# rgl-epfl/large-steps-pytorch

Measured on NVIDIA H100. Metric: from_differential solves/sec @1M verts, higher is better.
Workload: dtype f32

## Files before the change

include/largesteps_b200_diag.h:

```cpp
#ifndef LARGESTEPS_B200_DIAG_H
#define LARGESTEPS_B200_DIAG_H

#include "largesteps_b200.h"

#ifdef __cplusplus
extern "C" {
#endif

int ls_pcg_bench_spmm(void *handle, int k, int launches, void *stream);
int ls_pcg_bench(void **handles, int n_handles, int k, int which, int launches, void *stream);
int ls_pcg_batch_plan(int n, const int32_t *nslices, const int32_t *pat, int max_smem, int32_t *cluster, int32_t *res,
                      int32_t *group, int32_t *n_groups);
int ls_pcg_batch_plan_ex(int n, const int32_t *nslices, const int32_t *pat, const int32_t *cheb, int max_smem,
                         int32_t *cluster, int32_t *res, int32_t *group, int32_t *n_groups);
int ls_pcg_plan(int nslices, int k, int pat, int precond, int sm_count, int max_smem, int coop, int64_t *out8);
int ls_pcg_pattern_copy(void *handle, int64_t *info4, int32_t *poff, uint32_t *words, void *stream);
int ls_pcg_phase_cycles(void *handle, int64_t *out, int n , void *stream);

#ifdef __cplusplus
}
#endif
#endif
```

large-steps-pytorch_b200/csrc/ls_pcg.cu:

```cuda
#include <new>
#include <string.h>
#include <stdlib.h>
#include "ls_spmm_host.h"
#include "ls_sell_kernel.cuh"
#include "ls_pcg_fused.cuh"
#include "ls_fused_inst.h"

#ifndef LS_CLRES_DEFAULT
#define LS_CLRES_DEFAULT 0
#endif

namespace {

constexpr int KMAX = 4;
constexpr int VEC_THREADS = 256;
constexpr int CHUNK = 8;

struct PcgCtrl {
    double rz[KMAX], pAp[KMAX], rr[KMAX], bb[KMAX];
    float beta[KMAX];
    float rtol2;
    int maxit;
    int it;
    int done;
// ... 28 lines not shown
    int *desc_cnt;
    int *perm;
    int *inv;
    int *scan;
    int has_perm;
    int planned;
    int *soff;
    int2 *ent;
    long long sell_cap;
    long long sell_entries;
    int nslices;
    int sell_on;
    int sell_grid;
    int *poff;
    unsigned int *pcol;
    unsigned char *pcls;
    unsigned long long *pcls_tab;
    unsigned int *patmm;
    long long pat_cap;
    float offc;
    int pat_on;
    int pat_shared;
    int pat_stored;
    int pat_words;
    lsf::GridBar *gbar;
    double *partials;
    long long *dbg;
    unsigned long long *ring;
    int ring_slots;
    float *pv;
    float *z2, *cy, *cd;
    int cheb_m;
    float cheb_c0, cheb_c1[8], cheb_c2[8];
    float *gersh;
    struct FusedCfg : FusedPlan {
        int pat;
        const void *fn, *fn_prof;
    } fused[2];
    int max_smem_optin;
    int refine;
    float theta;
    int sell_tma;
    int sell_pf;
    cudaGraphExec_t graph[KMAX + 1];
    cudaStream_t cap_stream;
    int *pinned_done;
    cudaEvent_t ev[2];
    size_t ws_bytes;
};

static bool want_pattern() {
    const char *e = getenv("LS_PCG_PATTERN");
    return !(e && e[0] == '0');
}

struct Carve {
    size_t off = 0;
    size_t take(size_t bytes) {
        size_t o = off;
// ... 647 lines not shown
    return LS_OK;
}

const void *fused_fn(int K, int res, int nw, int pat, int sync, int prof, int cheb = 0) {
    if (cheb) return (K == 3 && !prof) ? ls_fused_fn_cheb(res, nw, pat, sync) : nullptr;
    if (K == 3 && !prof) return ls_fused_fn_jacobi(res, nw, pat, sync);
    return ls_fused_fn_misc(K, res, nw, pat, sync, prof);
}

static int env_int(const char *name, int dflt) {
    const char *e = getenv(name);
    return (e && e[0]) ? atoi(e) : dflt;
}

constexpr int CLRES_CS = 16;

struct PlanEnv {
    int graph;
    int cluster;
    int res;
    int onecta;
    int clres;
    int small_cta;
};

PlanEnv plan_env() {
    const char *mode = getenv("LS_PCG_MODE"), *small = getenv("LS_PCG_SMALLCTA");
    PlanEnv e;
    e.graph = mode && (mode[0] == 'g' || mode[0] == 'G');
    e.cluster = env_int("LS_PCG_CLUSTER", -1);
    e.res = env_int("LS_PCG_RES", -1);
    e.onecta = env_int("LS_PCG_ONECTA", lsf::PWARPS);
    e.clres = env_int("LS_PCG_CLRES", LS_CLRES_DEFAULT);
    e.small_cta = !(small && small[0] == '0');
    return e;
}

int slices_per_cta(int K, int res, int pat, int cheb, int sync, int max_smem) {
    if (res == 0) return 1 << 30;
    int n = 0;
    while (lsf::fused_smem_bytes(K, res, n + 1, pat, cheb, sync) <= (size_t)max_smem) ++n;
    return n;
}

int auto_precond(int nslices, int sm_count, int max_smem, const PlanEnv &env) {
    if (nslices <= env.onecta) return 1;
    if (env.cluster != 0 && nslices <= env.clres) return 1;
    const int g = sm_count < nslices ? sm_count : nslices;
    const int nsl_max = (nslices + g - 1) / g;
    const bool fits = lsf::fused_smem_bytes(3, 2, nsl_max, 0, 1, 0) + (size_t)nsl_max * 32 * 4 <= (size_t)max_smem;
    return fits ? 2 : 1;
}

FusedPlan plan_fused(int nslices, int K, int pat, int cheb, int sm_count, int max_smem, int coop, const PlanEnv &env) {
    FusedPlan p{};
    if (env.graph) return p;
    const int W = lsf::PWARPS;
// ... 9 lines not shown
        const bool res3 = cs == 1 && K == 3 && !cheb && nsl_max <= slices_per_cta(K, 3, pat, cheb, 1, max_smem);
        int res = (res3 && !(env.res >= 0 && env.res < 3)) ? 3 : 2;
        int nw = W;
        int cap4 = slices_per_cta(K, 4, pat, cheb, 1, max_smem);
        if (cap4 > 63) cap4 = 63;
        if (cs > 1 && !cheb && nsl_max <= cap4 && !(env.res >= 0 && env.res < 4)) {
            res = 4;
            if (K == 3 && nsl_max <= lsf::PT_SMALL / 32 && env.small_cta) nw = lsf::PT_SMALL / 32;
        }
        if (res == 4 && !fused_fn(K, res, nw, pat, 1, 0, cheb)) { res = 2; nw = W; }
        if (fused_fn(K, res, nw, pat, 1, 0, cheb)) return {1, cs, cs, res, nw, 1, nsl_max, lsf::fused_smem_bytes(K, res, nsl_max, pat, cheb, 1)};
    }
    if (!coop) return p;
    int g = sm_count < nslices ? sm_count : nslices;
    if (g > 255) g = 255;
    if (g < 1) g = 1;
    const int nsl_max = (nslices + g - 1) / g;
    int res = nsl_max <= slices_per_cta(K, 2, pat, cheb, 0, max_smem) ? 2 : (nsl_max <= slices_per_cta(K, 1, pat, cheb, 0, max_smem) ? 1 : 0);
    if (env.res >= 0 && env.res < res) res = env.res;
    int nw = W;
    if (K == 3 && res == 2 && nsl_max <= 16 && env.small_cta) nw = lsf::PT_SMALL / 32;
    if (!fused_fn(K, res, nw, pat, 0, 0, cheb)) return p;
    return {1, g, 0, res, nw, 0, nsl_max, lsf::fused_smem_bytes(K, res, nsl_max, pat, cheb, 0)};
}

cudaLaunchConfig_t cluster_launch(int grid, int cluster, int threads, size_t smem, cudaStream_t stream, cudaLaunchAttribute *at) {
    cudaLaunchConfig_t lc = {};
    lc.gridDim = dim3(grid);
    lc.blockDim = dim3(threads);
    lc.dynamicSmemBytes = smem;
    lc.stream = stream;
    at->id = cudaLaunchAttributeClusterDimension;
    at->val.clusterDim.x = cluster;
    at->val.clusterDim.y = 1;
    at->val.clusterDim.z = 1;
    lc.attrs = at;
    lc.numAttrs = 1;
    return lc;
}

bool device_accepts(const void *fn, const FusedPlan &p, const LsDevInfo &di) {
    bool ok = cudaFuncSetAttribute(fn, cudaFuncAttributeMaxDynamicSharedMemorySize, di.max_smem_optin) == cudaSuccess;
    if (ok && p.cluster > 8) ok = cudaFuncSetAttribute(fn, cudaFuncAttributeNonPortableClusterSizeAllowed, 1) == cudaSuccess;
    if (ok && p.cluster > 1) {
        cudaLaunchAttribute at;
        const cudaLaunchConfig_t lc = cluster_launch(p.grid, p.cluster, p.nw * 32, p.smem, 0, &at);
// ... 8 lines not shown
    return ok;
}

void configure_fused(PcgHandle *h, const LsDevInfo &di, const PlanEnv &env, int K, PcgHandle::FusedCfg *c) {
    memset(c, 0, sizeof(*c));
    if (!h->sell_on) return;
    const int cheb = (K == 3 && h->cheb_m > 1) ? 1 : 0;
    const int pat = (K == 3 && h->pat_on) ? 1 : 0;
    int coop = 0;
    if (cudaDeviceGetAttribute(&coop, cudaDevAttrCooperativeLaunch, di.device) != cudaSuccess) {
        coop = 0;
        cudaGetLastError();
    }
    auto kernel = [&](const FusedPlan &q, int prof) { return fused_fn(K, q.res, q.nw, pat, q.sync, prof, cheb); };
    FusedPlan p = plan_fused(h->nslices, K, pat, cheb, di.sm_count, di.max_smem_optin, coop, env);
    if (p.on && p.sync == 1 && !device_accepts(kernel(p, 0), p, di)) {
        PlanEnv grid_only = env;
        grid_only.cluster = 0;
        p = plan_fused(h->nslices, K, pat, cheb, di.sm_count, di.max_smem_optin, coop, grid_only);
    }
    if (!p.on || (p.sync == 0 && !device_accepts(kernel(p, 0), p, di))) return;
    static_cast<FusedPlan &>(*c) = p;
    c->pat = pat;
    c->fn = kernel(p, 0);
    c->fn_prof = kernel(p, 1);
    if (c->fn_prof) {
        cudaFuncSetAttribute(c->fn_prof, cudaFuncAttributeMaxDynamicSharedMemorySize, di.max_smem_optin);
        if (p.cluster > 8) cudaFuncSetAttribute(c->fn_prof, cudaFuncAttributeNonPortableClusterSizeAllowed, 1);
    }
    cudaGetLastError();
}

void fused_handle_args(const PcgHandle *h, int nsl_max, lsf::FusedArgs &a) {
    a.V = (int)h->V;
    a.Vp = h->Vp;
    a.nslices = h->nslices;
    a.nsl_max = nsl_max;
    a.soff = h->soff;
    a.ent = h->ent;
    a.poff = h->poff;
    a.pcol = h->pcol;
    a.pcls = h->pcls;
    a.pcls_tab = h->pcls_tab;
    a.offc = h->offc;
    a.pat_l1 = h->pat_shared;
    a.dinv = h->dinv;
// ... 2 lines not shown
    a.r = h->r;
    a.s = h->Ap;
    a.z = h->p;
    a.z2 = h->z2;
    a.cy = h->cy;
    a.cd = h->cd;
    a.perm = h->has_perm ? h->perm : nullptr;
    a.refine = h->refine;
    a.theta = h->theta;
    a.cheb_m = h->cheb_m;
    a.cheb_c0 = h->cheb_c0;
    for (int j = 0; j < 8; ++j) {
        a.cheb_c1[j] = h->cheb_c1[j];
        a.cheb_c2[j] = h->cheb_c2[j];
    }
}

int solve_fused(PcgHandle *h, const float *b, float *x, const float *x0, int k, float rtol, int maxit, float *info_dev,
                float *info_host, cudaStream_t stream) {
    PcgHandle::FusedCfg &c = h->fused[k == 4 ? 1 : 0];
    lsf::FusedArgs a{};
    fused_handle_args(h, c.nsl_max, a);
    a.kb = k;
    if (k == 4) a.cheb_m = 0;
    a.b = b;
    a.out = x;
    a.x0 = x0;
    a.rtol = rtol;
    a.maxit = maxit;
    a.bar = h->gbar;
    a.partials = h->partials;
    a.info = info_dev ? info_dev : h->info;
    const bool prof = getenv("LS_PCG_PROFILE") != nullptr && c.fn_prof != nullptr;
    a.dbg = prof ? h->dbg : nullptr;
    const void *fn = prof ? c.fn_prof : c.fn;
    void *params[] = {(void *)&a};
    cudaError_t ce;
    if (c.sync == 1) {
        if (c.cluster > 1) {
            cudaLaunchAttribute at;
            const cudaLaunchConfig_t lc = cluster_launch(c.grid, c.cluster, c.nw * 32, c.smem, stream, &at);
            ce = cudaLaunchKernelExC(&lc, fn, params);
        } else {
            ce = cudaLaunchKernel(fn, dim3(1), dim3(c.nw * 32), params, c.smem, stream);
        }
    } else {
// ... 306 lines not shown
            TRY_OR_FAIL(cudaGetLastError());
            lsk::pat_share_copy_kernel<<<2 * di.sm_count, 256, 0, stream>>>(ns, h->poff, h->pcol, npoff,
                                                                              reinterpret_cast<const unsigned int *>(h->p), soff2, stats, cap_scr);
            g_ls_launches.fetch_add(1);
            TRY_OR_FAIL(cudaGetLastError());
        }
        int hover = 1, hst[2] = {ns, 0}, hwords = 0;
        TRY_OR_FAIL(cudaMemcpyAsync(&hover, over, sizeof(int), cudaMemcpyDeviceToHost, stream));
        if (cap_scr > 0) {
            TRY_OR_FAIL(cudaMemcpyAsync(hst, stats, sizeof(int), cudaMemcpyDeviceToHost, stream));
            TRY_OR_FAIL(cudaMemcpyAsync(&hst[1], soff2 + ns, sizeof(int), cudaMemcpyDeviceToHost, stream));
        }
        TRY_OR_FAIL(cudaMemcpyAsync(&hwords, h->poff + ns, sizeof(int), cudaMemcpyDeviceToHost, stream));
        TRY_OR_FAIL(cudaStreamSynchronize(stream));
        h->pat_on = hover ? 0 : 1;
        h->pat_shared = (h->pat_on && cap_scr > 0 && lsk::pat_share_on(ns, hst[0], hst[1], cap_scr)) ? 1 : 0;
        h->pat_stored = h->pat_shared ? hst[0] : ns;
        h->pat_words = hwords;
        if (cap_scr > 0) {
            TRY_OR_FAIL(cudaMemsetAsync(h->r, 0, (size_t)((char *)(ptab + pmask + 1) - (char *)h->r), stream));
            if (lsk::pat_share_on(ns, hst[0], hst[1], cap_scr)) TRY_OR_FAIL(cudaMemsetAsync(h->p, 0, (size_t)hst[1] * 4, stream));
        }
    }
    h->cheb_m = 0;
    if (precond == 2 && hgersh > 0.f) {
        int m = env_int("LS_PCG_CHEB_M", 4);
        if (m < 2) m = 2;
        if (m > 8) m = 8;
        const double b = 1.02 * (double)hgersh, a = b / 30.0;
        const double th = 0.5 * (b + a), de = 0.5 * (b - a), sg = th / de;
        double rho = 1.0 / sg;
        h->cheb_c0 = (float)(1.0 / th);
        for (int j = 1; j < m; ++j) {
            const double rn = 1.0 / (2.0 * sg - rho);
            h->cheb_c1[j - 1] = (float)(rn * rho);
            h->cheb_c2[j - 1] = (float)(2.0 * rn / de);
            rho = rn;
        }
        h->cheb_m = m;
    }
    configure_fused(h, di, env, 3, &h->fused[0]);
    if (k_max >= 4) configure_fused(h, di, env, 4, &h->fused[1]);
    if (hflags & 8) {
        ls_set_error("perm_new2old is not a permutation of [0, V)");
        return fail(LS_ERR_BAD_ARG);
    }
// ... 165 lines not shown
    out8[0] = h->sell_on;
    out8[1] = h->sell_entries;
    out8[2] = h->sell_on ? h->sell_grid : h->spmm_grid;
    out8[3] = h->vec_grid;
    out8[4] = 0;
    out8[5] = 0;
    out8[6] = h->planned;
    out8[7] = h->has_perm;
    return LS_OK;
}

extern "C" int ls_pcg_plan(int nslices, int k, int pat, int precond, int sm_count, int max_smem, int coop, int64_t *out8) {
    LS_REQUIRE(out8 != nullptr, "out8 is NULL");
    LS_REQUIRE(nslices >= 1, "nslices must be positive");
    LS_REQUIRE(k == 3 || k == 4, "k must be 3 or 4 (the column counts of the fused kernel's instantiations)");
    LS_REQUIRE(precond >= 0 && precond <= 3, "precond must be 0 (none), 1 (Jacobi), 2 (Chebyshev polynomial over Jacobi) or 3 (auto)");
    LS_REQUIRE(sm_count >= 1 && max_smem > 0, "sm_count and max_smem must be positive");
    const PlanEnv env = plan_env();
    if (precond == 3) precond = auto_precond(nslices, sm_count, max_smem, env);
    const int cheb = (k == 3 && precond == 2) ? 1 : 0;
    const FusedPlan p = plan_fused(nslices, k, (k == 3 && pat) ? 1 : 0, cheb, sm_count, max_smem, coop ? 1 : 0, env);
    const int64_t o[8] = {p.on, p.grid, p.cluster, p.res, p.nw * 32, precond, (int64_t)p.smem, p.nsl_max};
    memcpy(out8, o, sizeof(o));
    return LS_OK;
}

extern "C" int ls_pcg_pattern_copy(void *handle, int64_t *info4, int32_t *poff, uint32_t *words, void *stream_) {
    PcgHandle *h = (PcgHandle *)handle;
    LS_REQUIRE(h != nullptr && info4 != nullptr, "NULL pointer");
    info4[0] = h->pat_on;
    info4[1] = h->nslices;
    info4[2] = h->pat_on ? h->pat_stored : 0;
    info4[3] = h->pat_on ? h->pat_words : 0;
    if (h->pat_on && poff != nullptr && words != nullptr) {
        cudaStream_t stream = (cudaStream_t)stream_;
        LS_CUDA_TRY(cudaMemcpyAsync(poff, h->poff, (size_t)(h->nslices + 1) * 4, cudaMemcpyDeviceToHost, stream));
        LS_CUDA_TRY(cudaMemcpyAsync(words, h->pcol, (size_t)h->pat_words * 4, cudaMemcpyDeviceToHost, stream));
        LS_CUDA_TRY(cudaStreamSynchronize(stream));
    }
    return LS_OK;
}

extern "C" int64_t ls_pcg_spmm_bytes(void *handle, int k) {
    PcgHandle *h = (PcgHandle *)handle;
    if (!h) return 0;
    return 8 * h->nnz + 4 * (h->V + 1) + 8 * (int64_t)k * h->V;
// ... 261 lines not shown
```

large-steps-pytorch_b200/csrc/ls_pcg_fused.cuh:

```cuda
#pragma once
#include <cuda_bf16.h>
#include <type_traits>
#include "ls_common.cuh"
#include "ls_sell_kernel.cuh"

#ifndef LS_RING_SOA
#define LS_RING_SOA 0
#endif
#ifndef LS_XP4
#define LS_XP4 0
#endif
#ifndef LS_FHADD
#define LS_FHADD 0
#endif
#ifndef LS_Z_EL
#define LS_Z_EL 0
#endif
#ifndef LS_XP_STREAM
#define LS_XP_STREAM 0
#endif
#ifndef LS_POLL_FENCE
#define LS_POLL_FENCE 0
#endif

namespace lsf {

#ifndef LS_PT
#define LS_PT 768
#endif
constexpr int PT = LS_PT;
constexpr int PWARPS = PT / 32;
constexpr int PT_SMALL = 256;
constexpr int NVMAX = 16;

struct GridBar {
    unsigned int count;
    unsigned int gen;
};

__device__ __forceinline__ unsigned int ld_acquire(const unsigned int *p) {
    unsigned int v;
    asm volatile("ld.acquire.gpu.global.u32 %0, [%1];" : "=r"(v) : "l"(p) : "memory");
    return v;
}
__device__ __forceinline__ float4 ld_coherent4(const float *p) {
    float4 v;
// ... 78 lines not shown
    allreduce_finish<NV>(v, partials, gb, gen, parity, red, G);
}

__device__ __forceinline__ int exp2_of(double d) { return (int)((__double_as_longlong(d) >> 52) & 0x7ff) - 1023; }

template <int KCOL, int N>
__device__ __forceinline__ double pick_lane(const double (&v)[N], int off, int lane) {
    double d = 0.0;
#pragma unroll
    for (int i = 0; i < KCOL; ++i) {
        double t = v[off + i];
        asm volatile("" : "+d"(t));
        if (lane == i) d = t;
    }
    return d;
}

struct FusedArgs {
    int V;
    long long Vp;
    int nslices;
    int nsl_max;
    int kb;
    const int *soff;
    const int2 *ent;
    const int *poff;
    const unsigned int *pcol;
    const unsigned char *pcls;
    const unsigned long long *pcls_tab;
    float offc;
    int pat_l1;
    const float *dinv;
    float *x;
    float *pv;
    float *r;
    float *s;
    float *z;
    float *z2;
    float *cy, *cd;
    int cheb_m;
    float cheb_c0;
    float cheb_c1[8], cheb_c2[8];
    const float *b;
    float *out;
    const float *x0;
    const int *perm;
// ... 297 lines not shown
constexpr size_t FUSED_SMEM_HDR = 4096 + 1024;
constexpr size_t FUSED_BATCH_ARGS = 4352 + 320;
__host__ __device__ inline size_t fused_off_bytes(int nsl_max) { return ((size_t)(2 * (nsl_max + 1)) * 4 + 127) / 128 * 128; }

__host__ __device__ inline int fused_row_bytes(int K, int res, int pat, int cheb = 0) {
    if (res == 0) return 0;
    return 4 * ((res == 1 ? 2 * K : (res == 2 ? 4 * K : 4 * K + 4)) + ((cheb && res == 2) ? 2 * K : 0)) + (pat ? 1 : 4);
}
__host__ __device__ inline size_t fused_tab_bytes(int pat) { return pat ? (size_t)lsk::PAT_CLASSES * 8 : 0; }
__host__ __device__ inline size_t fused_cl_bytes(int sync) { return sync == 1 ? (size_t)(2 * NVMAX * 16 * 8) : 0; }
inline size_t fused_smem_bytes(int K, int res, int nsl_max, int pat, int cheb, int sync) {
    return FUSED_SMEM_HDR + fused_cl_bytes(sync) + fused_off_bytes(nsl_max) + fused_tab_bytes(pat) + (size_t)nsl_max * 32u * fused_row_bytes(K, res, pat, cheb);
}

template <int K, int RES, int NW, bool PAT, int SYNC, bool PROF, bool CHEB = false, bool ZH = false, bool BATCH = false>
__global__ void __launch_bounds__(NW * 32, 1) pcg_fused_kernel(const typename FusedParam<BATCH>::type prm) {
    static_assert(K == 3 || K == 4, "z rows are float4");
    static_assert(!ZH || (K == 3 && !CHEB && RES != 3), "bf16 rows: 3 columns, Jacobi, published through global or distributed shared memory");
    static_assert(RES != 4 || (SYNC == 1 && !CHEB), "cluster-resident rows: one cluster, Jacobi");
    static_assert(!BATCH || (K == 3 && SYNC == 1 && !PROF && (RES == 2 || (RES == 3 && !CHEB))),
                  "batch: one cluster per mesh, 3 columns; Jacobi at RES 3 or 2, Chebyshev at RES 2");
    static_assert(sizeof(Scal) <= FUSED_BATCH_ARGS - 4352 && FUSED_BATCH_ARGS + sizeof(FusedArgs) <= FUSED_SMEM_HDR, "header layout");
    constexpr bool KEEP = (SYNC == 1);
    extern __shared__ __align__(16) unsigned char smem_raw[];
    const FusedArgs &a = kernel_args(prm, smem_raw + FUSED_BATCH_ARGS);
    const bool pkeep = KEEP || (PAT && a.pat_l1 != 0);
    double *red = reinterpret_cast<double *>(smem_raw);
    Scal *S = reinterpret_cast<Scal *>(smem_raw + 4352);
    double *cl = reinterpret_cast<double *>(smem_raw + FUSED_SMEM_HDR);
    int *off_s = reinterpret_cast<int *>(smem_raw + FUSED_SMEM_HDR + fused_cl_bytes(SYNC));
    const int nsl_max = a.nsl_max;
    int *poff_s = off_s + (nsl_max + 1);
    float *tab_d = reinterpret_cast<float *>(reinterpret_cast<unsigned char *>(off_s) + fused_off_bytes(nsl_max));
    float *tab_p = tab_d + lsk::PAT_CLASSES;
    float *r_s = tab_d + (PAT ? 2 * lsk::PAT_CLASSES : 0);
    float *s_s = r_s + (size_t)nsl_max * K * 32;
    float *d_s = s_s + (size_t)nsl_max * K * 32;
    unsigned char *c_s = reinterpret_cast<unsigned char *>(d_s);
    float *x_s = d_s + (size_t)(RES >= 1 ? nsl_max : 0) * (PAT ? 8 : 32);
    float *p_s = x_s + (size_t)nsl_max * K * 32;
    float *z_s = p_s + (size_t)nsl_max * K * 32;
    float *cy_s = z_s;
    float *cd_s = cy_s + (size_t)nsl_max * K * 32;

    const int tid = threadIdx.x, lane = tid & 31, warp = tid >> 5;
    const int G = BATCH ? (int)cluster_nctarank() : (int)gridDim.x, cta = BATCH ? (int)ClusterSync::rank() : (int)blockIdx.x;
    const int s_begin = (RES == 4) ? min(cta * nsl_max, a.nslices) : (int)((long long)a.nslices * cta / G);
    const int s_end = (RES == 4) ? min(s_begin + nsl_max, a.nslices) : (int)((long long)a.nslices * (cta + 1) / G);
    const long long Vp = a.Vp;
    const int kb = a.kb;
    constexpr int U = PAT ? 4 : 8;

    typename std::conditional<SYNC == 1, ClusterSync, GridSync>::type sync;
    if constexpr (SYNC == 1) {
        sync.cl = cl;
        sync.parity = 0;
        sync.G = G;
        sync.red = red;
        sync.S = S;
    } else {
        sync.bar = a.bar;
        sync.partials = a.partials;
        sync.ring = a.ring;
        sync.ring_slots = a.ring_slots;
        sync.gen = 0;
        sync.parity = 0;
        sync.G = G;
        sync.red = red;
        sync.S = S;
    }

    auto R = [&](int li, int k, int row) -> float & { return RES ? r_s[((size_t)li * K + k) * 32 + lane] : a.r[(size_t)k * Vp + row]; };
    auto Sv = [&](int li, int k, int row) -> float & { return RES ? s_s[((size_t)li * K + k) * 32 + lane] : a.s[(size_t)k * Vp + row]; };
    constexpr bool XP4 = (RES == 1) && (LS_XP4 != 0);
// ... 218 lines not shown
                        for (int k = 0; k < K; ++k) w_[k] = fmaf(wv, xk[k], w_[k]);
                    }
                }
                for (int j = U; j < w; j += U) {
#pragma unroll
                    for (int u = 0; u < U; ++u) cv[u] = (j + u < w) ? ld_ent<KEEP>(e + (j + u) * 32) : make_int2(row, 0);
                    float4 xv[U];
#pragma unroll
                    for (int u = 0; u < U; ++u) xv[u] = ZldP(cv[u].x);
#pragma unroll
                    for (int u = 0; u < U; ++u) {
                        const float wv = __int_as_float(cv[u].y);
                        const float xk[4] = {xv[u].x, xv[u].y, xv[u].z, xv[u].w};
                        if (cv[u].x == row) zo = xv[u];
#pragma unroll
                        for (int k = 0; k < K; ++k) w_[k] = fmaf(wv, xk[k], w_[k]);
                    }
                }
            }
            epi(li, row, w_, zo);
        }
    };

    auto own_z = [&](int li, int row) -> float4 {
        if constexpr (CHEB) {
            if constexpr (RES == 2) return make_float4(CY(li, 0), CY(li, 1), CY(li, 2), K > 3 ? CY(li, K > 3 ? 3 : 0) : 0.f);
            else return Zld(row);
        } else if constexpr (RES >= 1) {
            const float di_ = Dv(li, row);
            if constexpr (ZH) return unpack_bf16_row(pack_bf16_row(di_ * R(li, 0, row), di_ * R(li, 1, row), di_ * R(li, 2, row)));
            else return make_float4(di_ * R(li, 0, row), di_ * R(li, 1, row), di_ * R(li, 2, row), K > 3 ? di_ * R(li, K > 3 ? 3 : 0, row) : 0.f);
        } else {
            return ZldP(row);
        }
    };

    auto cheb_first = [&]() {
        for (int s = s_begin + warp; s < s_end; s += NW) {
            const int li = s - s_begin, row = s * 32 + lane;
            const float di = Dv(li, row) * a.cheb_c0;
            float yy[4] = {0.f, 0.f, 0.f, 0.f};
#pragma unroll
            for (int k = 0; k < K; ++k) {
                yy[k] = di * R(li, k, row);
                if constexpr (RES == 2) CY(li, k) = yy[k];
                CD(li, k, row) = yy[k];
            }
            Zst(row, make_float4(yy[0], yy[1], yy[2], yy[3]));
        }
    };
    auto cheb_steps = [&](double (&acc2)[2 * K]) {
// ... 20 lines not shown
                    for (int k = 0; k < K; ++k) {
                        const float rk = R(li, k, row);
                        const float dn = fmaf(c1, dprev[k], c2 * (di * (rk - t[k])));
                        yy[k] = yk[k] + dn;
                        CD(li, k, row) = dn;
                        if constexpr (RES == 2) CY(li, k) = yy[k];
                        if (last) {
                            acc2[k] += (double)rk * (double)yy[k];
                            acc2[K + k] += (double)rk * (double)rk;
                        }
                    }
                    *reinterpret_cast<float4 *>(zalt + 4 * (size_t)row) = make_float4(yy[0], yy[1], yy[2], yy[3]);
                });
            float *tz = zcur;
            zcur = zalt;
            zalt = tz;
        }
    };

    auto cold_init = [&]() {
        double acc[2 * K];
#pragma unroll
        for (int i = 0; i < 2 * K; ++i) acc[i] = 0.0;
        for (int s = s_begin + warp; s < s_end; s += NW) {
            const int li = s - s_begin, row = s * 32 + lane;
            float di = 0.f, bv[K];
#pragma unroll
            for (int k = 0; k < K; ++k) bv[k] = 0.f;
            if (row < a.V) {
                di = a.dinv[row];
                const long long io = a.perm ? a.perm[row] : row;
#pragma unroll
                for (int k = 0; k < K; ++k)
                    if (k < kb) bv[k] = a.b[io * kb + k];
            }
            if (RES && !PAT) d_s[(size_t)li * 32 + lane] = di;
            float zz[4] = {0.f, 0.f, 0.f, 0.f};
#pragma unroll
            for (int k = 0; k < K; ++k) zz[k] = di * bv[k];
            ZstP(row, zz);
#pragma unroll
            for (int k = 0; k < K; ++k) {
                R(li, k, row) = bv[k];
                Sv(li, k, row) = 0.f;
                X(li, k, row) = 0.f;
                P(li, k, row) = 0.f;
// ... 70 lines not shown
                    for (int k = 0; k < K; ++k) {
                        ax[k] = fma((double)wv, (double)xk[k], ax[k]);
                        fl[k] = fmaf(fabsf(wv), fabsf(xk[k]), fl[k]);
                    }
                }
            }
            float di = 0.f, bv[K];
#pragma unroll
            for (int k = 0; k < K; ++k) bv[k] = 0.f;
            if (row < a.V) {
                di = a.dinv[row];
                const long long io = a.perm ? a.perm[row] : row;
#pragma unroll
                for (int k = 0; k < K; ++k)
                    if (k < kb) bv[k] = a.b[io * kb + k];
            }
            if (RES && !PAT) d_s[(size_t)li * 32 + lane] = di;
#pragma unroll
            for (int k = 0; k < K; ++k) {
                const float rv = (float)((double)bv[k] - ax[k]);
                R(li, k, row) = rv;
                float zz = di * rv;
                if constexpr (ZH) zz = __bfloat162float(__float2bfloat16_rn(zz));
                acc[k] += (double)rv * (double)zz;
                acc[K + k] += (double)rv * (double)rv;
                acc[2 * K + k] += (double)fl[k] * (double)fl[k];
                acc[3 * K + k] += (double)bv[k] * (double)bv[k];
            }
        }
        if constexpr (CHEB) {
            if (cheb_m > 1) {
                double a2[2 * K];
#pragma unroll
                for (int i = 0; i < 2 * K; ++i) a2[i] = 0.0;
                sync.barrier();
                cheb_first();
                cheb_steps(a2);
#pragma unroll
                for (int k = 0; k < K; ++k) acc[k] = a2[k];
            }
        }
        sync.template allreduce_slow<4 * K>(acc);
        if (tid == 0) {
            const double rtol2 = (double)a.rtol * (double)a.rtol;
            const double th = (double)a.theta * 5.9604644775390625e-08;
            int all = 1, worse = 0, bad = 0;
            for (int k = 0; k < K; ++k) {
                const double gam = acc[k], rr = acc[K + k], fl2 = acc[2 * K + k], bb = acc[3 * K + k];
                if (warm) {
                    S->bb[k] = bb;
// ... 20 lines not shown
                if (!all && !bad) S->restarts += 1;
            }
            if (bad) S->status = 3;
            else if (all) S->status = 1;
            else if (S->it >= a.maxit) S->status = 2;
            else S->status = 0;
            S->stop = S->status != 0;
        }
        __syncthreads();
        if (S->cold) return;
        if (!S->stop) {
            for (int s = s_begin + warp; s < s_end; s += NW) {
                const int li = s - s_begin, row = s * 32 + lane;
                const float di = Dv(li, row);
                float zz[4] = {0.f, 0.f, 0.f, 0.f};
#pragma unroll
                for (int k = 0; k < K; ++k) {
                    zz[k] = di * R(li, k, row);
                    if (warm) {
                        Sv(li, k, row) = 0.f;
                        P(li, k, row) = 0.f;
                    }
                }
                if (cheb_m <= 1)
                    ZstP(row, zz);
            }
            sync.barrier();
        }
    };

    if (a.x0 != nullptr) {
        for (int s = s_begin + warp; s < s_end; s += NW) {
            const int li = s - s_begin, row = s * 32 + lane;
            float xv[K];
#pragma unroll
            for (int k = 0; k < K; ++k) xv[k] = 0.f;
            if (row < a.V) {
                const long long io = a.perm ? a.perm[row] : row;
#pragma unroll
                for (int k = 0; k < K; ++k)
                    if (k < kb) xv[k] = a.x0[io * kb + k];
            }
#pragma unroll
            for (int k = 0; k < K; ++k) X(li, k, row) = xv[k];
        }
        restart_from_x(true);
        if (S->cold) {
// ... 85 lines not shown
                    if (lane == 0 && anybad) S->status = 3;
                };
                sync.template allreduce<K, K, false>(dacc, S->e_dl, S->skipA, true, postA);
                if (prof) { const long long t1 = clock64(); tS2 += t1 - t0; t0 = t1; }
            }
            {
                float alpha[K];
#pragma unroll
                for (int k = 0; k < K; ++k) alpha[k] = S->alpha[k];
                double acc2[2 * K];
#pragma unroll
                for (int i = 0; i < 2 * K; ++i) acc2[i] = 0.0;
                bool preconditioned = false;
                if constexpr (CHEB) {
                    if (cheb_m > 1) {
                        for (int s = s_begin + warp; s < s_end; s += NW) {
                            const int li = s - s_begin, row = s * 32 + lane;
#pragma unroll
                            for (int k = 0; k < K; ++k) R(li, k, row) = fmaf(-alpha[k], Sv(li, k, row), R(li, k, row));
                        }
                        __syncwarp();
                        cheb_first();
                        cheb_steps(acc2);
                        preconditioned = true;
                    }
                }
                if (!preconditioned)
                for (int s = s_begin + warp; s < s_end; s += NW) {
                    const int li = s - s_begin, row = s * 32 + lane;
                    const float di = Dv(li, row);
                    float zz[4] = {0.f, 0.f, 0.f, 0.f}, rn[K];
#pragma unroll
                    for (int k = 0; k < K; ++k) {
                        rn[k] = fmaf(-alpha[k], Sv(li, k, row), R(li, k, row));
                        R(li, k, row) = rn[k];
                        zz[k] = di * rn[k];
                    }
                    ZstP(row, zz);
#pragma unroll
                    for (int k = 0; k < K; ++k) {
                        acc2[k] += (double)(rn[k] * zz[k]);
                        acc2[K + k] += (double)(rn[k] * rn[k]);
                    }
                }
                if (prof) { const long long t1 = clock64(); tB += t1 - t0; t0 = t1; }
                auto postB = [&](const double gn, const double rrn) {
// ... 92 lines not shown
```

large-steps-pytorch_b200/largesteps_b200/_native.py:

```python
import ctypes
import os
from ctypes import c_int, c_int32, c_int64, c_uint32, c_uint64, c_size_t, c_float, c_void_p, c_char_p, POINTER

import numpy as np
import torch

_HERE = os.path.dirname(os.path.abspath(__file__))
LIB_PATH = os.environ.get("LS_LIB_PATH") or os.path.join(_HERE, "libls_b200.so")

LS_OK, LS_ERR_BAD_ARG, LS_ERR_CUDA, LS_ERR_BREAKDOWN, LS_ERR_NOT_CONVERGED, LS_ERR_UNSUPPORTED, \
    LS_ERR_INDEX_RANGE, LS_ERR_WORKSPACE = range(8)

SYMBOLS = {
    "ls_version": (c_int, []),
    "ls_last_error": (c_char_p, []),
    "ls_status_string": (c_char_p, [c_int]),
    "ls_launch_count": (c_uint64, []),
    "ls_assemble_workspace_bytes": (c_int, [c_int64, c_int64, POINTER(c_size_t)]),
    "ls_assemble_count": (c_int, [c_void_p, c_int, c_int64, c_int64, c_void_p, c_size_t, POINTER(c_int64), c_void_p]),
    "ls_assemble_fill": (c_int, [c_void_p, c_int, c_void_p, c_int64, c_int64, c_int, c_float, c_float,
                                 c_void_p, c_size_t, c_int64, c_void_p, c_void_p, c_void_p,
                                 c_void_p, c_void_p, c_void_p, c_void_p]),
    "ls_coo_to_csr": (c_int, [c_void_p, c_void_p, c_int64, c_int64, c_void_p, c_void_p, c_void_p]),
    "ls_spmm_csr_f32": (c_int, [c_int64, c_void_p, c_void_p, c_void_p, c_void_p, c_int64, c_void_p, c_int64, c_int, c_void_p]),
# ... 1 lines not shown
    "ls_pcg_create": (c_int, [POINTER(c_void_p), c_int64, c_int64, c_void_p, c_void_p, c_void_p, c_void_p, c_int, c_int,
                              c_void_p, c_size_t, c_void_p]),
    "ls_order_workspace_bytes": (c_int, [c_int64, POINTER(c_size_t)]),
    "ls_order_morton": (c_int, [c_void_p, c_int64, c_void_p, c_void_p, c_size_t, c_void_p]),
    "ls_pcg_solve": (c_int, [c_void_p, c_void_p, c_void_p, c_void_p, c_int, c_float, c_int, c_void_p,
                             POINTER(c_float), c_void_p]),
    "ls_pcg_destroy": (c_int, [c_void_p]),
    "ls_pcg_set_refinement": (c_int, [c_void_p, c_int, c_float]),
    "ls_pcg_bench_spmm": (c_int, [c_void_p, c_int, c_int, c_void_p]),
    "ls_pcg_spmm_bytes": (c_int64, [c_void_p, c_int]),
    "ls_pcg_describe": (c_int, [c_void_p, POINTER(c_int64)]),
    "ls_pcg_bench": (c_int, [POINTER(c_void_p), c_int, c_int, c_int, c_int, c_void_p]),
    "ls_pcg_phase_cycles": (c_int, [c_void_p, POINTER(c_int64), c_int, c_void_p]),
    "ls_pcg_pattern_copy": (c_int, [c_void_p, POINTER(c_int64), POINTER(c_int32), POINTER(c_uint32), c_void_p]),
    "ls_pcg_batch_create": (c_int, [POINTER(c_void_p), POINTER(c_void_p), c_int, c_void_p]),
    "ls_pcg_batch_solve": (c_int, [c_void_p, c_void_p, c_void_p, c_void_p, c_int, c_float, c_int, c_void_p,
                                   POINTER(c_float), c_void_p]),
    "ls_pcg_batch_destroy": (c_int, [c_void_p]),
    "ls_pcg_batch_plan": (c_int, [c_int, POINTER(c_int32), POINTER(c_int32), c_int, POINTER(c_int32), POINTER(c_int32),
                                  POINTER(c_int32), POINTER(c_int32)]),
    "ls_pcg_batch_plan_ex": (c_int, [c_int, POINTER(c_int32), POINTER(c_int32), POINTER(c_int32), c_int, POINTER(c_int32),
                                     POINTER(c_int32), POINTER(c_int32), POINTER(c_int32)]),
    "ls_pcg_plan": (c_int, [c_int, c_int, c_int, c_int, c_int, c_int, c_int, POINTER(c_int64)]),
    "ls_glue_scratch_bytes": (c_int, [POINTER(c_size_t)]),
    "ls_bucket_workspace_bytes": (c_int, [c_int64, POINTER(c_size_t)]),
    "ls_face_incidence": (c_int, [c_void_p, c_int, c_int64, c_int64, c_void_p, c_void_p, c_void_p, c_size_t, c_void_p]),
    "ls_index_buckets": (c_int, [c_void_p, c_int, c_int64, c_int64, c_void_p, c_void_p, c_void_p, c_size_t, c_void_p]),
    "ls_gather_rows_f32": (c_int, [c_void_p, c_void_p, c_int, c_int64, c_int, c_void_p, c_void_p]),
    "ls_gather_rows_bwd_f32": (c_int, [c_void_p, c_void_p, c_void_p, c_int64, c_int, c_void_p, c_void_p]),
    "ls_face_normals_f32": (c_int, [c_void_p, c_void_p, c_int, c_int64, c_void_p, c_void_p]),
    "ls_face_normals_bwd_f32": (c_int, [c_void_p, c_void_p, c_int, c_int64, c_int64, c_void_p, c_void_p, c_void_p, c_void_p, c_void_p]),
    "ls_vertex_normals_f32": (c_int, [c_void_p, c_void_p, c_int, c_int64, c_int64, c_void_p, c_void_p, c_void_p, c_void_p, c_void_p,
                                      c_void_p, c_void_p, c_void_p]),
    "ls_vertex_normals_bwd_f32": (c_int, [c_void_p, c_void_p, c_int, c_int64, c_int64, c_void_p, c_void_p, c_void_p, c_void_p, c_void_p,
                                          c_void_p, c_void_p, c_void_p, c_void_p, c_void_p, c_void_p]),
    "ls_massmatrix_voronoi_f32": (c_int, [c_void_p, c_void_p, c_int, c_int64, c_int64, c_void_p, c_void_p, c_void_p, c_void_p]),
    "ls_massmatrix_voronoi_bwd_f32": (c_int, [c_void_p, c_void_p, c_int, c_int64, c_int64, c_void_p, c_void_p, c_void_p,
                                              c_void_p, c_void_p]),
    "ls_vertex_normals_batch_scratch_bytes": (c_int, [c_int, POINTER(c_size_t)]),
    "ls_vertex_normals_batch_f32": (c_int, [c_void_p, c_void_p, c_int, c_int64, c_int64, c_int, c_void_p, c_void_p,
                                            c_void_p, c_void_p, c_void_p, c_void_p, c_void_p, c_void_p, c_void_p, c_void_p,
                                            c_void_p, c_size_t, c_void_p]),
    "ls_vertex_normals_batch_bwd_f32": (c_int, [c_void_p, c_void_p, c_int, c_int64, c_int64, c_int, c_void_p, c_void_p,
                                                c_void_p, c_void_p, c_void_p, c_void_p, c_void_p, c_void_p, c_void_p, c_void_p,
                                                c_void_p, c_void_p, c_void_p, c_void_p, c_size_t, c_void_p]),
    "ls_adam_uniform_step": (c_int, [c_void_p, c_void_p, c_void_p, c_void_p, c_int64, c_float, c_float, c_float,
# ... 75 lines not shown
```

large-steps-pytorch_b200/largesteps_b200/solvers.py:

```python
import ctypes
import warnings

import numpy as np

import torch
from torch.autograd import Function

from . import _native as N
from .geometry import csr_of, order_of

K_MAX = 4
PRECOND = {"none": 0, "jacobi": 1, "chebyshev": 2, "auto": 3}


class Solver:

    def __init__(self, M):
        pass

    def solve(self, b, backward=False):
        raise NotImplementedError()


class PCGSolver(Solver):
# ... 81 lines not shown
        self._sync_info()
        self._unreported = False
        return int(self._info_host[1])

    @property
    def restarts(self):
        self._sync_info()
        return int(self._info_host[6])

    def raise_for_status(self):
        st = self.status
        if st == 3:
            raise N.Breakdown(f"CG breakdown after {self.iterations} iterations (matrix not SPD or NaN in the right-hand side)")
        if st == 2:
            raise N.NotConverged(f"PCG did not reach rtol={self.rtol} within maxit={self.maxit} (relres {self.relres})")

    def describe(self):
        out = (ctypes.c_int64 * 8)()
        N.check(N.lib().ls_pcg_describe(self._handle, out), "ls_pcg_describe")
        o = [int(v) for v in out]
        pat = self.pattern_copy()
        pat = {"pattern_slices": pat["slices"], "pattern_slices_stored": pat["stored"], "pattern_column_bytes": 4 * pat["words"]}
        if o[4] >= 10:
            return {"algo": "fused", "sell_engine": o[0], "sell_entries": o[1], "grid": o[2], "cluster": o[3],
                    "residency": o[4] - 10, "precond": {0: "none", 1: "jacobi", 2: "chebyshev"}.get(o[5], o[5]), "threads": o[6],
                    "reordered": o[7],
                    "persistent": 2 if o[4] - 10 >= 1 else 1, "persistent_grid": o[2], **pat}
        keys = ("sell_engine", "sell_entries", "spmm_grid", "vec_grid", "persistent", "persistent_grid", "planned", "reordered")
        d = dict(zip(keys, o))
        d["algo"] = "graph"
        d.update(pat)
        return d

    def pattern_copy(self, arrays=False):
        info = (ctypes.c_int64 * 4)()
        N.check(N.lib().ls_pcg_pattern_copy(self._handle, info, None, None, None), "ls_pcg_pattern_copy")
        d = dict(zip(("on", "slices", "stored", "words"), [int(v) for v in info]))
        if arrays and d["on"]:
            poff = np.zeros(d["slices"] + 1, np.int32)
            words = np.zeros(max(d["words"], 1), np.uint32)
            with torch.cuda.device(self.device):
                N.check(N.lib().ls_pcg_pattern_copy(self._handle, info, poff.ctypes.data_as(ctypes.POINTER(ctypes.c_int32)),
                                                    words.ctypes.data_as(ctypes.POINTER(ctypes.c_uint32)), N.stream_ptr(self.device)),
                        "ls_pcg_pattern_copy")
            d["poff"], d["words_array"] = poff, words[:d["words"]]
        return d

    def phase_cycles(self, per_cta=False):
        g = self.describe()["persistent_grid"] if per_cta else 0
# ... 77 lines not shown
    with torch.cuda.device(dev):
        N.check(N.lib().ls_pcg_bench(arr, len(solvers), k, which, launches, N.stream_ptr(dev)), "ls_pcg_bench")


def workspace_bytes(V, nnz):
    nbytes = ctypes.c_size_t(0)
    N.check(N.lib().ls_pcg_workspace_bytes(int(V), int(nnz), K_MAX, ctypes.byref(nbytes)), "ls_pcg_workspace_bytes")
    return nbytes.value


def plan(nslices, pattern, sm_count, max_smem, precond="jacobi", k=3, cooperative=True):
    if precond not in PRECOND:
        raise ValueError(f"Unknown preconditioner '{precond}'.")
    out = (ctypes.c_int64 * 8)()
    N.check(N.lib().ls_pcg_plan(int(nslices), int(k), 1 if pattern else 0, PRECOND[precond], int(sm_count), int(max_smem),
                                1 if cooperative else 0, out), "ls_pcg_plan")
    on, grid, cluster, res, threads, pc = (int(v) for v in out[:6])
    if not on:
        return {"algo": "graph"}
    return {"algo": "fused", "grid": grid, "cluster": cluster, "residency": res, "threads": threads,
            "precond": {0: "none", 1: "jacobi", 2: "chebyshev"}[pc]}


class CholeskySolver(PCGSolver):

    def __init__(self, M, workspace=None):
        super().__init__(M, rtol=1e-7, maxit=10000, precond="auto", warm_start=False, check=False, refine=1,
                         workspace=workspace)


class ConjugateGradientSolver(PCGSolver):

    def __init__(self, M, workspace=None):
        super().__init__(M, rtol=1e-7, maxit=10000, precond="auto", warm_start=True, workspace=workspace)


class DifferentiableSolve(Function):

    @staticmethod
    def forward(ctx, solver, b):
        ctx.solver = solver
        return solver.solve(b, backward=False)

    @staticmethod
    def backward(ctx, grad_output):
        solver_grad = None
# ... 8 lines not shown
```

Baseline: 476.2.

## Add block-local first-order Neumann preconditioner for diagonally dominant fused PCG

Adds a local Neumann-series preconditioner, z = D r − c·D²·(offdiag_local r), computed from residuals held in each CTA's shared memory. It applies only to the fused cooperative kernel at residency 1 with pattern-compressed columns, Jacobi preconditioning and a Gershgorin check confirming diagonal dominance. The aim is to cut PCG iteration count at 1M vertices. The cost is an extra local SpMV-like pass per iteration and a host sync at setup for the Gershgorin bound, and convergence may change because the preconditioner is block-local.

```diff
diff --git a/include/largesteps_b200_diag.h b/include/largesteps_b200_diag.h
--- a/include/largesteps_b200_diag.h
+++ b/include/largesteps_b200_diag.h
@@ -14,6 +14,9 @@
 int ls_pcg_batch_plan_ex(int n, const int32_t *nslices, const int32_t *pat, const int32_t *cheb, int max_smem,
                          int32_t *cluster, int32_t *res, int32_t *group, int32_t *n_groups);
 int ls_pcg_plan(int nslices, int k, int pat, int precond, int sm_count, int max_smem, int coop, int64_t *out8);
+int ls_pcg_plan_local_neumann(int nslices, int k, int pat, int precond, int sm_count, int max_smem, int coop, int dominant,
+                              int32_t *on);
+int ls_pcg_local_neumann(void *handle, int32_t *on);
 int ls_pcg_pattern_copy(void *handle, int64_t *info4, int32_t *poff, uint32_t *words, void *stream);
 int ls_pcg_phase_cycles(void *handle, int64_t *out, int n , void *stream);
 
diff --git a/large-steps-pytorch_b200/csrc/ls_pcg.cu b/large-steps-pytorch_b200/csrc/ls_pcg.cu
--- a/large-steps-pytorch_b200/csrc/ls_pcg.cu
+++ b/large-steps-pytorch_b200/csrc/ls_pcg.cu
@@ -74,6 +74,7 @@
     int pat_on;
     int pat_shared;
     int pat_stored;
+    int diag_dom;
     int pat_words;
     lsf::GridBar *gbar;
     double *partials;
@@ -87,6 +88,7 @@
     float *gersh;
     struct FusedCfg : FusedPlan {
         int pat;
+        int local_neu;
         const void *fn, *fn_prof;
     } fused[2];
     int max_smem_optin;
@@ -780,6 +782,7 @@
     int onecta;
     int clres;
     int small_cta;
+    int localneu;
 };
 
 PlanEnv plan_env() {
@@ -791,6 +794,7 @@
     e.onecta = env_int("LS_PCG_ONECTA", lsf::PWARPS);
     e.clres = env_int("LS_PCG_CLRES", LS_CLRES_DEFAULT);
     e.small_cta = !(small && small[0] == '0');
+    e.localneu = env_int("LS_PCG_LOCALNEU", 1) != 0;
     return e;
 }
 
@@ -846,6 +850,11 @@
     if (K == 3 && res == 2 && nsl_max <= 16 && env.small_cta) nw = lsf::PT_SMALL / 32;
     if (!fused_fn(K, res, nw, pat, 0, 0, cheb)) return p;
     return {1, g, 0, res, nw, 0, nsl_max, lsf::fused_smem_bytes(K, res, nsl_max, pat, cheb, 0)};
+}
+
+int local_neumann_on(const FusedPlan &p, int K, int pat, int jacobi, int max_smem, int dominant, const PlanEnv &env) {
+    return (env.localneu && p.on && p.sync == 0 && p.res == 1 && K == 3 && pat && jacobi && dominant &&
+            p.nsl_max > slices_per_cta(K, 2, pat, 0, 0, max_smem)) ? 1 : 0;
 }
 
 cudaLaunchConfig_t cluster_launch(int grid, int cluster, int threads, size_t smem, cudaStream_t stream, cudaLaunchAttribute *at) {
@@ -900,6 +909,7 @@
     if (!p.on || (p.sync == 0 && !device_accepts(kernel(p, 0), p, di))) return;
     static_cast<FusedPlan &>(*c) = p;
     c->pat = pat;
+    c->local_neu = local_neumann_on(p, K, pat, h->precond != 0 && !cheb, di.max_smem_optin, h->diag_dom, env);
     c->fn = kernel(p, 0);
     c->fn_prof = kernel(p, 1);
     if (c->fn_prof) {
@@ -948,6 +958,7 @@
     lsf::FusedArgs a{};
     fused_handle_args(h, c.nsl_max, a);
     a.kb = k;
+    a.local_neu = c.local_neu;
     if (k == 4) a.cheb_m = 0;
     a.b = b;
     a.out = x;
@@ -1300,6 +1311,19 @@
             if (lsk::pat_share_on(ns, hst[0], hst[1], cap_scr)) TRY_OR_FAIL(cudaMemsetAsync(h->p, 0, (size_t)hst[1] * 4, stream));
         }
     }
+    h->diag_dom = 0;
+    if (h->pat_on) {
+        float g = hgersh;
+        if (precond != 2) {
+            TRY_OR_FAIL(cudaMemsetAsync(h->gersh, 0, 64, stream));
+            k_gershgorin<<<(unsigned)((V + 255) / 256), 256, 0, stream>>>(V, h->rowptr, h->col, h->val, h->gersh);
+            g_ls_launches.fetch_add(1);
+            TRY_OR_FAIL(cudaGetLastError());
+            TRY_OR_FAIL(cudaMemcpyAsync(&g, h->gersh, sizeof(float), cudaMemcpyDeviceToHost, stream));
+            TRY_OR_FAIL(cudaStreamSynchronize(stream));
+        }
+        h->diag_dom = (g > 0.f && g < 2.f) ? 1 : 0;
+    }
     h->cheb_m = 0;
     if (precond == 2 && hgersh > 0.f) {
         int m = env_int("LS_PCG_CHEB_M", 4);
@@ -1511,6 +1535,28 @@
     const FusedPlan p = plan_fused(nslices, k, (k == 3 && pat) ? 1 : 0, cheb, sm_count, max_smem, coop ? 1 : 0, env);
     const int64_t o[8] = {p.on, p.grid, p.cluster, p.res, p.nw * 32, precond, (int64_t)p.smem, p.nsl_max};
     memcpy(out8, o, sizeof(o));
+    return LS_OK;
+}
+
+extern "C" int ls_pcg_local_neumann(void *handle, int32_t *on) {
+    PcgHandle *h = (PcgHandle *)handle;
+    LS_REQUIRE(h != nullptr && on != nullptr, "NULL pointer");
+    *on = h->fused[0].on ? h->fused[0].local_neu : 0;
+    return LS_OK;
+}
+
+extern "C" int ls_pcg_plan_local_neumann(int nslices, int k, int pat, int precond, int sm_count, int max_smem, int coop, int dominant,
+                                         int32_t *on) {
+    LS_REQUIRE(on != nullptr, "on is NULL");
+    LS_REQUIRE(nslices >= 1, "nslices must be positive");
+    LS_REQUIRE(k == 3 || k == 4, "k must be 3 or 4 (the column counts of the fused kernel's instantiations)");
+    LS_REQUIRE(precond >= 0 && precond <= 3, "precond must be 0 (none), 1 (Jacobi), 2 (Chebyshev polynomial over Jacobi) or 3 (auto)");
+    LS_REQUIRE(sm_count >= 1 && max_smem > 0, "sm_count and max_smem must be positive");
+    const PlanEnv env = plan_env();
+    if (precond == 3) precond = auto_precond(nslices, sm_count, max_smem, env);
+    const int cheb = (k == 3 && precond == 2) ? 1 : 0, p3 = (k == 3 && pat) ? 1 : 0;
+    const FusedPlan p = plan_fused(nslices, k, p3, cheb, sm_count, max_smem, coop ? 1 : 0, env);
+    *on = local_neumann_on(p, k, p3, precond == 1, max_smem, dominant ? 1 : 0, env);
     return LS_OK;
 }
 
diff --git a/large-steps-pytorch_b200/csrc/ls_pcg_fused.cuh b/large-steps-pytorch_b200/csrc/ls_pcg_fused.cuh
--- a/large-steps-pytorch_b200/csrc/ls_pcg_fused.cuh
+++ b/large-steps-pytorch_b200/csrc/ls_pcg_fused.cuh
@@ -22,6 +22,12 @@
 #ifndef LS_POLL_FENCE
 #define LS_POLL_FENCE 0
 #endif
+#ifndef LS_LOCALNEU_CHECK
+#define LS_LOCALNEU_CHECK 0
+#endif
+#if LS_LOCALNEU_CHECK
+#include <cassert>
+#endif
 
 namespace lsf {
 
@@ -146,6 +152,7 @@
     int nslices;
     int nsl_max;
     int kb;
+    int local_neu;
     const int *soff;
     const int2 *ent;
     const int *poff;
@@ -489,6 +496,7 @@
                   "batch: one cluster per mesh, 3 columns; Jacobi at RES 3 or 2, Chebyshev at RES 2");
     static_assert(sizeof(Scal) <= FUSED_BATCH_ARGS - 4352 && FUSED_BATCH_ARGS + sizeof(FusedArgs) <= FUSED_SMEM_HDR, "header layout");
     constexpr bool KEEP = (SYNC == 1);
+    constexpr bool LOCAL_NEU = PAT && RES == 1 && SYNC == 0 && K == 3 && !CHEB && !BATCH && ZH;
     extern __shared__ __align__(16) unsigned char smem_raw[];
     const FusedArgs &a = kernel_args(prm, smem_raw + FUSED_BATCH_ARGS);
     const bool pkeep = KEEP || (PAT && a.pat_l1 != 0);
@@ -517,6 +525,7 @@
     const long long Vp = a.Vp;
     const int kb = a.kb;
     constexpr int U = PAT ? 4 : 8;
+    const bool lneu = LOCAL_NEU && a.local_neu != 0;
 
     typename std::conditional<SYNC == 1, ClusterSync, GridSync>::type sync;
     if constexpr (SYNC == 1) {
@@ -781,11 +790,68 @@
         }
     };
 
+    auto local_pass = [&](auto &acc) {
+        unsigned int dm = 0x7f800000u;
+        for (int i = lane; i < lsk::PAT_CLASSES; i += 32) {
+            const float d = tab_d[i];
+            if (d > 0.f && d < 3.0e38f) dm = min(dm, __float_as_uint(d));
+        }
+        const float dmin = __uint_as_float(__reduce_min_sync(0xffffffffu, dm));
+        const float kc = dmin < 3.0e38f ? -(dmin * dmin) * a.offc : 0.f;
+        const int lo = s_begin * 32;
+        const unsigned int nrows = (unsigned int)(s_end - s_begin) * 32u;
+        for (int s = s_begin + warp; s < s_end; s += NW) {
+            const int li = s - s_begin, row = s * 32 + lane;
+            const lsk::PatSlice ps = lsk::pat_slice(poff_s + li);
+            float nb[K];
+#pragma unroll
+            for (int k = 0; k < K; ++k) nb[k] = 0.f;
+            auto add_owned = [&](int col) {
+#if LS_LOCALNEU_CHECK
+                assert(col >= 0 && col < a.nslices * 32);
+#endif
+                const unsigned int lj = (unsigned int)(col - lo);
+                if (col != row && lj < nrows) {
+#if LS_LOCALNEU_CHECK
+                    assert(lj < (unsigned int)nsl_max * 32u);
+#endif
+                    const unsigned int sl = lj >> 5, ln = lj & 31u;
+#pragma unroll
+                    for (int k = 0; k < K; ++k) nb[k] += r_s[((size_t)sl * K + k) * 32 + ln];
+                }
+            };
+            for (int m = 0; m < ps.w2; m += U) {
+                int2 raw[U];
+#pragma unroll
+                for (int u = 0; u < U; ++u) raw[u] = lsk::pat_load(a.pcol, ps, m + u, row, lane, pkeep);
+#pragma unroll
+                for (int u = 0; u < U; ++u) {
+                    const int2 c = lsk::pat_cols(raw[u], ps.wide, row);
+                    add_owned(c.x);
+                    add_owned(c.y);
+                }
+            }
+            const float di = Dv(li, row);
+            float zz[4] = {0.f, 0.f, 0.f, 0.f}, rv[K];
+#pragma unroll
+            for (int k = 0; k < K; ++k) {
+                rv[k] = R(li, k, row);
+                zz[k] = fmaf(kc, nb[k], di * rv[k]);
+            }
+            ZstP(row, zz);
+#pragma unroll
+            for (int k = 0; k < K; ++k) acc[k] += (double)rv[k] * (double)zz[k];
+        }
+    };
+
     auto own_z = [&](int li, int row) -> float4 {
         if constexpr (CHEB) {
             if constexpr (RES == 2) return make_float4(CY(li, 0), CY(li, 1), CY(li, 2), K > 3 ? CY(li, K > 3 ? 3 : 0) : 0.f);
             else return Zld(row);
         } else if constexpr (RES >= 1) {
+            if constexpr (LOCAL_NEU) {
+                if (lneu) return ZldP(row);
+            }
             const float di_ = Dv(li, row);
             if constexpr (ZH) return unpack_bf16_row(pack_bf16_row(di_ * R(li, 0, row), di_ * R(li, 1, row), di_ * R(li, 2, row)));
             else return make_float4(di_ * R(li, 0, row), di_ * R(li, 1, row), di_ * R(li, 2, row), K > 3 ? di_ * R(li, K > 3 ? 3 : 0, row) : 0.f);
@@ -852,6 +918,35 @@
         double acc[2 * K];
 #pragma unroll
         for (int i = 0; i < 2 * K; ++i) acc[i] = 0.0;
+        bool published = false;
+        if constexpr (LOCAL_NEU) {
+            if (lneu) {
+                for (int s = s_begin + warp; s < s_end; s += NW) {
+                    const int li = s - s_begin, row = s * 32 + lane;
+                    float bv[K];
+#pragma unroll
+                    for (int k = 0; k < K; ++k) bv[k] = 0.f;
+                    if (row < a.V) {
+                        const long long io = a.perm ? a.perm[row] : row;
+#pragma unroll
+                        for (int k = 0; k < K; ++k)
+                            if (k < kb) bv[k] = a.b[io * kb + k];
+                    }
+#pragma unroll
+                    for (int k = 0; k < K; ++k) {
+                        R(li, k, row) = bv[k];
+                        Sv(li, k, row) = 0.f;
+                        X(li, k, row) = 0.f;
+                        P(li, k, row) = 0.f;
+                        acc[K + k] += (double)bv[k] * (double)bv[k];
+                    }
+                }
+                __syncthreads();
+                local_pass(acc);
+                published = true;
+            }
+        }
+        if (!published)
         for (int s = s_begin + warp; s < s_end; s += NW) {
             const int li = s - s_begin, row = s * 32 + lane;
             float di = 0.f, bv[K];
@@ -968,10 +1063,16 @@
                 R(li, k, row) = rv;
                 float zz = di * rv;
                 if constexpr (ZH) zz = __bfloat162float(__float2bfloat16_rn(zz));
-                acc[k] += (double)rv * (double)zz;
+                if (!lneu) acc[k] += (double)rv * (double)zz;
                 acc[K + k] += (double)rv * (double)rv;
                 acc[2 * K + k] += (double)fl[k] * (double)fl[k];
                 acc[3 * K + k] += (double)bv[k] * (double)bv[k];
+            }
+        }
+        if constexpr (LOCAL_NEU) {
+            if (lneu) {
+                __syncthreads();
+                local_pass(acc);
             }
         }
         if constexpr (CHEB) {
@@ -1038,7 +1139,7 @@
                         P(li, k, row) = 0.f;
                     }
                 }
-                if (cheb_m <= 1)
+                if (cheb_m <= 1 && !lneu)
                     ZstP(row, zz);
             }
             sync.barrier();
@@ -1170,6 +1271,22 @@
                         __syncwarp();
                         cheb_first();
                         cheb_steps(acc2);
+                        preconditioned = true;
+                    }
+                }
+                if constexpr (LOCAL_NEU) {
+                    if (lneu) {
+                        for (int s = s_begin + warp; s < s_end; s += NW) {
+                            const int li = s - s_begin, row = s * 32 + lane;
+#pragma unroll
+                            for (int k = 0; k < K; ++k) {
+                                const float rn = fmaf(-alpha[k], Sv(li, k, row), R(li, k, row));
+                                R(li, k, row) = rn;
+                                acc2[K + k] += (double)(rn * rn);
+                            }
+                        }
+                        __syncthreads();
+                        local_pass(acc2);
                         preconditioned = true;
                     }
                 }
diff --git a/large-steps-pytorch_b200/largesteps_b200/_native.py b/large-steps-pytorch_b200/largesteps_b200/_native.py
--- a/large-steps-pytorch_b200/largesteps_b200/_native.py
+++ b/large-steps-pytorch_b200/largesteps_b200/_native.py
@@ -47,6 +47,8 @@
     "ls_pcg_batch_plan_ex": (c_int, [c_int, POINTER(c_int32), POINTER(c_int32), POINTER(c_int32), c_int, POINTER(c_int32),
                                      POINTER(c_int32), POINTER(c_int32), POINTER(c_int32)]),
     "ls_pcg_plan": (c_int, [c_int, c_int, c_int, c_int, c_int, c_int, c_int, POINTER(c_int64)]),
+    "ls_pcg_plan_local_neumann": (c_int, [c_int, c_int, c_int, c_int, c_int, c_int, c_int, c_int, POINTER(c_int32)]),
+    "ls_pcg_local_neumann": (c_int, [c_void_p, POINTER(c_int32)]),
     "ls_glue_scratch_bytes": (c_int, [POINTER(c_size_t)]),
     "ls_bucket_workspace_bytes": (c_int, [c_int64, POINTER(c_size_t)]),
     "ls_face_incidence": (c_int, [c_void_p, c_int, c_int64, c_int64, c_void_p, c_void_p, c_void_p, c_size_t, c_void_p]),
diff --git a/large-steps-pytorch_b200/largesteps_b200/solvers.py b/large-steps-pytorch_b200/largesteps_b200/solvers.py
--- a/large-steps-pytorch_b200/largesteps_b200/solvers.py
+++ b/large-steps-pytorch_b200/largesteps_b200/solvers.py
@@ -127,9 +127,11 @@
         pat = self.pattern_copy()
         pat = {"pattern_slices": pat["slices"], "pattern_slices_stored": pat["stored"], "pattern_column_bytes": 4 * pat["words"]}
         if o[4] >= 10:
+            ln = ctypes.c_int32(0)
+            N.check(N.lib().ls_pcg_local_neumann(self._handle, ctypes.byref(ln)), "ls_pcg_local_neumann")
             return {"algo": "fused", "sell_engine": o[0], "sell_entries": o[1], "grid": o[2], "cluster": o[3],
                     "residency": o[4] - 10, "precond": {0: "none", 1: "jacobi", 2: "chebyshev"}.get(o[5], o[5]), "threads": o[6],
-                    "reordered": o[7],
+                    "reordered": o[7], "local_neumann": int(ln.value),
                     "persistent": 2 if o[4] - 10 >= 1 else 1, "persistent_grid": o[2], **pat}
         keys = ("sell_engine", "sell_entries", "spmm_grid", "vec_grid", "persistent", "persistent_grid", "planned", "reordered")
         d = dict(zip(keys, o))
@@ -253,6 +255,16 @@
             "precond": {0: "none", 1: "jacobi", 2: "chebyshev"}[pc]}
 
 
+def plan_local_neumann(nslices, pattern, sm_count, max_smem, precond="jacobi", k=3, cooperative=True, dominant=True):
+    if precond not in PRECOND:
+        raise ValueError(f"Unknown preconditioner '{precond}'.")
+    on = ctypes.c_int32(0)
+    N.check(N.lib().ls_pcg_plan_local_neumann(int(nslices), int(k), 1 if pattern else 0, PRECOND[precond], int(sm_count),
+                                              int(max_smem), 1 if cooperative else 0, 1 if dominant else 0, ctypes.byref(on)),
+            "ls_pcg_plan_local_neumann")
+    return int(on.value)
+
+
 class CholeskySolver(PCGSolver):
 
     def __init__(self, M, workspace=None):
```

Result: faster. 488.2, median of 6 (+2.5%).
